# mcx/AgileRL

Hardware: AMD Instinct MI355X
Metric: population env-steps/sec + learner updates/sec, 8-agent PPO at 1/2/4/8 MI355X (higher is better)
Workload: dtype f32 (GAE carry f64); 1 GPU; config 2: one 8-agent PPO population sharded 8 agents per GPU, 128 vec envs per agent, T=16, batch 128, 4 epochs, MLP enc[64]->64 + heads[64] (shared encoder), tournament every 5 iterations; population=8, pop_per_gpu=8, num_envs=128, learn_step=2048, batch_size=128, update_epochs=4, learner=fused, parallelism=population-sharded x1

## Files before the change

agilerl_amd/csrc/learner.hip:

```cpp
#include <cmath>
#include <cstdlib>
#include <type_traits>

#include "agx_common.h"
#include "rollout.h"

namespace agx {

#ifndef AGX_LEARN_UNIFORM
#define AGX_LEARN_UNIFORM 1
#endif
#ifndef AGX_LEARN_RS2
#define AGX_LEARN_RS2 0
#endif
#ifndef AGX_LEARN_B2_TAGGED
#define AGX_LEARN_B2_TAGGED 1
#endif
#ifndef AGX_LEARN_B2_SWEEP1
#define AGX_LEARN_B2_SWEEP1 1
#endif
#ifndef AGX_LEARN_VEC_EARLY
#define AGX_LEARN_VEC_EARLY 1
#endif
#ifndef AGX_LEARN_STORE1
#define AGX_LEARN_STORE1 1
#endif

constexpr int kNT = 512;
constexpr int kNW = kNT / kWave;
constexpr int kSB = 32;
constexpr int kMaxSlot = 10;
constexpr int kMaxK = 16;
constexpr int kMaxPT = 32;
constexpr int kMaxA = 16;
constexpr int kMaxBlk = 28;

constexpr int kB2Words = 2 * kNW * kMaxK + 2;
constexpr size_t b2_words_off(size_t P) { return ((4 + kMaxK) * P + 1 + 3) / 4 * 4; }
typedef __attribute__((address_space(1))) unsigned long long gu64;

typedef unsigned v4u __attribute__((ext_vector_type(4)));

struct NetDims {
    int D, A, ne, eo[3], ha, hc;
};

struct Blk {
    int f0, len, rowlen, l0, ldst;
};

struct LearnPlan {
    int ok;
    int D, A, ne, ein[3], eout[3], eaff[3], lat, ha, hc, H, n;
    int f_ew[3], f_eb[3], f_eg[3], f_ebe[3];
    int f_aw, f_ab, f_ag, f_abe, f_aow, f_aob, f_cw, f_cb, f_cg, f_cbe, f_cow, f_cob;
    int l_ew[3], l_eld[3], l_eb[3], l_eg[3], l_ebe[3];
    int l_hw, l_hld, l_hb, l_hg, l_hbe;
    int l_aow, l_aold, l_aob, l_cow, l_cold, l_cob;
    int param_end;
    int l_x0, ld_x0, l_xe[3], ld_xe[3], l_re[3], l_xh, ld_xh, l_rh;
    int l_s1, l_s2, ld_s;
    int l_lg, l_dlg, l_dvb, l_val, l_row;
    int l_red, red_e[3], red_h, l_stat, l_stamp, l_b2x;
    int l_grad;
    int lds_floats, act_floats;
    int slab;
    int nt[6], ncol[6], slot0[6], nslot[6], nslots;
    int nblk;
    Blk blk[kMaxBlk];
};

constexpr int rup(int x, int m) { return (x + m - 1) / m * m; }

constexpr LearnPlan make_plan(NetDims d) {
    LearnPlan pl{};
    pl.ok = 0;
    pl.D = d.D;
    pl.A = d.A;
// ... 188 lines not shown
    if constexpr (W == 32)
        v = fmaxf(v, __builtin_bit_cast(float, __builtin_amdgcn_ds_swizzle(__builtin_bit_cast(int, v), 0x401f)));
    if constexpr (W == 64) {
        v = fmaxf(v, bcast<0x142, 0xa>(v, -__builtin_huge_valf()));
        v = fmaxf(v, bcast<0x143, 0xc>(v, -__builtin_huge_valf()));
        v = readlane_f(v, 63);
    }
    return v;
}
template <int W>
__device__ __forceinline__ int wrow(int lane, int wave) {
    return W == 64 ? wave : (W == 32 ? wave * 2 + (lane >> 5) : wave + kNW * (lane >> 4));
}
template <int SB>
constexpr int m_tiles() { return SB < 16 ? 1 : SB / 16; }
__device__ __forceinline__ float rowgroup_sum(float v) {
    v += __builtin_bit_cast(float, __builtin_amdgcn_ds_swizzle(__builtin_bit_cast(int, v), 0x401f));
    const int l = (int)(threadIdx.x & 63);
    return v + __builtin_bit_cast(float, __builtin_amdgcn_ds_bpermute((l ^ 32) << 2, __builtin_bit_cast(int, v)));
}
template <class T>
__device__ __forceinline__ T *in_vgpr(T *ptr) {
    asm volatile("" : "+v"(ptr));
    return ptr;
}
template <class T>
__device__ __forceinline__ T *to_sgpr(T *ptr) {
    const unsigned long long u = reinterpret_cast<unsigned long long>(ptr);
    const unsigned lo = __builtin_amdgcn_readfirstlane((unsigned)u);
    const unsigned hi = __builtin_amdgcn_readfirstlane((unsigned)(u >> 32));
    return reinterpret_cast<T *>(((unsigned long long)hi << 32) | lo);
}
__device__ __forceinline__ int vlane() {
    int v = (int)threadIdx.x;
    asm volatile("" : "+v"(v));
    return v & 63;
}
__device__ __forceinline__ int vtid() {
    int v = (int)threadIdx.x;
    asm volatile("" : "+v"(v));
    return v;
}
__device__ __forceinline__ int swave() {
    int w = __builtin_amdgcn_readfirstlane((int)threadIdx.x >> 6);
    asm volatile("" : "+s"(w));
    return w;
}
#define AGX_IDS                                             \
    const int lane = vlane(), wave = swave();               \
    const int lr16 = lane & 15, lq = lane >> 4;             \
    const int rrow = wave + kNW * lq, sub = lr16;           \
    (void)lr16, (void)lq, (void)rrow, (void)sub, (void)lane

__device__ __forceinline__ void block_sum2(float &a, float &b, float *stat, int slot, int lane, int wave) {
    a = row_sum(a);
    b = row_sum(b);
    const float wa = readlane_f(a, 0) + readlane_f(a, 16) + readlane_f(a, 32) + readlane_f(a, 48);
    const float wb = readlane_f(b, 0) + readlane_f(b, 16) + readlane_f(b, 32) + readlane_f(b, 48);
    if (lane == 0) {
        stat[slot * kNW + wave] = wa;
        stat[(slot + 1) * kNW + wave] = wb;
    }
    __syncthreads();
    float ta = 0.f, tb = 0.f;
    for (int i = 0; i < kNW; ++i) {
        ta += stat[slot * kNW + i];
        tb += stat[(slot + 1) * kNW + i];
    }
    a = ta;
    b = tb;
}

#ifndef AGX_MFMA_KB
#define AGX_MFMA_KB 16
#endif
template <int K, class FA, class FB>
__device__ __forceinline__ f4 mfma_tile(f4 acc, FA a, FB b) {
    const int lane = vlane();
    const int r = lane & 15, q = lane >> 4;
    constexpr int KB = K < AGX_MFMA_KB ? K : AGX_MFMA_KB;
    constexpr int NB = K / KB;
    static_assert(K % KB == 0 && KB % 4 == 0, "k batches");
    float av[2][KB / 4], bv[2][KB / 4];
#pragma unroll
    for (int j = 0; j < KB / 4; ++j) {
        av[0][j] = a(r, 4 * j + q);
        bv[0][j] = b(4 * j + q, r);
    }
#pragma unroll
    for (int i = 0; i < NB; ++i) {
        if (i + 1 < NB) {
#pragma unroll
            for (int j = 0; j < KB / 4; ++j) {
                av[(i + 1) & 1][j] = a(r, (i + 1) * KB + 4 * j + q);
                bv[(i + 1) & 1][j] = b((i + 1) * KB + 4 * j + q, r);
            }
        }
        __builtin_amdgcn_sched_barrier(0);
#pragma unroll
        for (int j = 0; j < KB / 4; ++j)
            acc = __builtin_amdgcn_mfma_f32_16x16x4f32(av[i & 1][j], bv[i & 1][j], acc, 0, 0, 0);
        __builtin_amdgcn_sched_barrier(0);
    }
    return acc;
}

template <class C>
__device__ __forceinline__ int flat_to_lds(int f) {
    constexpr LearnPlan pl = C::plan;
    int l = 0;
#pragma unroll
    for (int b = 0; b < pl.nblk; ++b) {
        constexpr int dummy = 0;
        (void)dummy;
        const Blk k = pl.blk[b];
        if (f >= k.f0 && f < k.f0 + k.len) {
            const int i = f - k.f0;
            l = k.l0 + (i / k.rowlen) * k.ldst + i % k.rowlen;
        }
    }
    return l;
}
template <class C>
// ... 223 lines not shown
#if AGX_LEARN_UNIFORM
    const int cs = (n4s + g.K - 1) / g.K;
    int oc0 = kk * cs < n4s ? kk * cs : n4s, oc1 = oc0 + cs < n4s ? oc0 + cs : n4s;
    const float inv_cs = 1.f / (float)cs;
#else
    int oc0 = n4s * kk / g.K, oc1 = n4s * (kk + 1) / g.K;
#endif
    int pc1 = oc1 < n4 ? oc1 : n4;
    constexpr int kUsed4 = JN > 0 ? JN : (n4 + kNT - 1) / kNT;
    static_assert(pl.param_end % 4 == 0 && pl.slab >= pl.param_end + 4 + 2 * kNW * kMaxK, "sum slab layout");
    static_assert(4 * kUsed4 <= kMaxPT, "owned slots");
    auto own_c = [&](int j) { return oc0 + vtid() + kNT * j; };
    const int jn_own = __builtin_amdgcn_readfirstlane((oc1 - oc0 + kNT - 1) / kNT);
    asm volatile("" : "+v"(oc0), "+v"(oc1), "+v"(pc1));
    float am[kMaxPT], av[kMaxPT];
    unsigned gbits = 0, vbits = 0;
#pragma unroll
    for (int i = 0; i < kMaxPT; ++i) {
        if (i >= 4 * kUsed4) {
            am[i] = av[i] = 0.f;
            continue;
        }
        const int c = own_c(i >> 2), l = 4 * c + (i & 3);
        int grp = 0;
        const int f = c < pc1 ? lds_to_flat<C>(l, grp) : -1;
        am[i] = f >= 0 ? gm[f] : 0.f;
        av[i] = f >= 0 ? gv[f] : 0.f;
        if (f >= 0) vbits |= 1u << i;
        if (grp) gbits |= 1u << i;
    }
    asm volatile("" : "+v"(vbits), "+v"(gbits));
    __syncthreads();

    constexpr int nmb_dummy = 0;
    (void)nmb_dummy;
    const int Bp = g.batch_p ? g.batch_p[p] : g.B;
    const int Ep = g.epochs_p ? g.epochs_p[p] : g.E;
    const float entp = g.ent_p ? g.ent_p[p] : g.ent;
    const int nmb = (int)((S + Bp - 1) / Bp);
    float loss_total = 0.f;
    double kl_total = 0.0;
    int n_done = 0, epochs_done = 0;
    const long long step0 = *step_v;
    double pb1 = pow((double)g.b1, (double)step0), pb2 = pow((double)g.b2, (double)step0);
    const float lr_p = g.lr[p];
    float *rowf = sm + pl.l_row;
    float *stat = sm + pl.l_stat;
    int *acts = reinterpret_cast<int *>(sm + pl.l_row + 4 * kSB);
    unsigned *legal = reinterpret_cast<unsigned *>(sm + pl.l_row + 5 * kSB);
    if (g.debug_stall && p == 0 && kk == 1) return;

    constexpr int kPreObs = (SB * pl.D + kNT - 1) / kNT;
    constexpr bool kPrefetch = kPreObs == 1;
    struct Pre {
        int e, mb, sb;
        float ob[kPreObs];
        unsigned rv;
    };
    const bool has_mask = g.gmask != nullptr;
    const int tid0 = vtid();
    const int rw_rr = tid0 < 4 * kSB ? tid0 % kSB : (tid0 < 5 * kSB ? tid0 - 4 * kSB : tid0 - 5 * kSB);
    const bool rw_on = tid0 < 6 * kSB;
    const unsigned *rw0 = in_vgpr(tid0 < 4 * kSB ? reinterpret_cast<const unsigned *>(g.grow) + ((size_t)p * 4 + tid0 / kSB) * S
                                  : (tid0 < 5 * kSB || !has_mask) ? reinterpret_cast<const unsigned *>(g.gact) + (size_t)p * S
                                                                   : g.gmask + (size_t)p * S);
    const size_t rw_es = (size_t)g.P * S * (tid0 < 4 * kSB ? 4 : 1);
    const float *ob0 = in_vgpr(g.gobs + (size_t)p * S * pl.D);
    const size_t ob_es = (size_t)g.P * S * pl.D;
    auto fetch = [&](int e_, int mb_, int sb_) {
        Pre r;
        r.e = e_;
        r.mb = mb_;
        r.sb = sb_;
        const int tid = vtid();
        const long long s0_ = (long long)mb_ * Bp;
        const int bsz_ = (int)((s0_ + Bp <= S) ? Bp : S - s0_);
        const int nrow_ = e_ >= Ep ? 0 : (bsz_ - sb_ < SB ? bsz_ - sb_ : SB);
        const size_t ee = (size_t)(e_ < Ep ? e_ : 0);
        const size_t row0 = (size_t)(s0_ + sb_);
        const float *eo = ob0 + ee * ob_es;
#pragma unroll
        for (int k = 0; k < kPreObs; ++k) {
            const int i = tid + k * kNT;
            r.ob[k] = eo[i < nrow_ * pl.D ? row0 * pl.D + i : 0];
        }
        r.rv = rw0[ee * rw_es + ((rw_on && rw_rr < nrow_) ? row0 + rw_rr : 0)];
        return r;
    };
    Pre pre{};
    if constexpr (kPrefetch) pre = fetch(0, 0, kk * SB);

    bool local = false;
    if (g.K > 1) {
        unsigned *xc = g.cnt + 3 * g.P + 1 + (size_t)p * kMaxK;
        if (tid == 0) {
            int x;
            asm volatile("s_getreg_b32 %0, hwreg(HW_REG_XCC_ID)" : "=s"(x));
            __hip_atomic_store(xc + kk, (unsigned)(x & 15) + 1u, __ATOMIC_RELAXED, __HIP_MEMORY_SCOPE_AGENT);
            asm volatile("s_waitcnt vmcnt(0)" ::: "memory");
            unsigned *ctr = g.cnt + 2 * g.P + 1 + p;
            __hip_atomic_fetch_add(ctr, 1u, __ATOMIC_RELAXED, __HIP_MEMORY_SCOPE_AGENT);
            unsigned spins = 0;
            int ok = 1;
            while (__hip_atomic_load(ctr, __ATOMIC_RELAXED, __HIP_MEMORY_SCOPE_AGENT) < (unsigned)g.K) {
                __builtin_amdgcn_s_sleep(1);
                if (++spins > kSpinMax) {
                    __hip_atomic_store(tmo_v, 1u, __ATOMIC_RELAXED, __HIP_MEMORY_SCOPE_AGENT);
                    if (err_v) __hip_atomic_fetch_or(err_v, 1u, __ATOMIC_RELAXED, __HIP_MEMORY_SCOPE_AGENT);
                    ok = 0;
                    break;
                }
            }
            stat[4 * kNW] = ok ? 1.f : 0.f;
        }
        __syncthreads();
        if (stat[4 * kNW] == 0.f) return;
        const int ln = vlane();
        const unsigned v = ln < g.K ? __hip_atomic_load(xc + ln, __ATOMIC_RELAXED, __HIP_MEMORY_SCOPE_AGENT) : 0u;
        const unsigned v0 = __builtin_amdgcn_readlane(v, 0);
        bool same = v0 != 0u;
        for (int q = 1; q < g.K; ++q) same = same && __builtin_amdgcn_readlane(v, q) == v0;
        local = same && !g.write_through;
    }

    float *slab_p = in_vgpr(g.slabs + (g.K > 1 ? (size_t)p * 2 * g.K * pl.slab : 0));
    float *sum_p = in_vgpr(g.sums + (g.K > 1 ? (size_t)p * 2 * pl.slab : 0));
    unsigned *ctr1 = in_vgpr(g.cnt + p);
    unsigned *ctr2 = in_vgpr(g.cnt + g.P + 1 + p);
    unsigned *ctr3 = in_vgpr(g.cnt + 3 * g.P + 1 + (size_t)g.P * kMaxK + p);
#if AGX_LEARN_B2_TAGGED
    unsigned long long *b2_p =
        in_vgpr(reinterpret_cast<unsigned long long *>(g.cnt + b2_words_off(g.P)) + (size_t)p * 2 * kB2Words);
    (void)ctr2;
#endif
    for (int e = 0; e < Ep; ++e) {
        for (int mb = 0; mb < nmb; ++mb) {
            const long long s0 = (long long)mb * Bp;
            const int bsz = (int)((s0 + Bp <= S) ? Bp : S - s0);
            const float inv_b = 1.f / (float)bsz;
            const int tid = vtid();
            f4 acc[kMaxSlot];
#pragma unroll
            for (int s = 0; s < kMaxSlot; ++s) acc[s] = f4{0.f, 0.f, 0.f, 0.f};
            const bool single = AGX_LEARN_STORE1 && kk * SB < bsz && kk * SB + g.K * SB >= bsz;
            if (!single)
                for (int i = tid; i < pl.l_stat - pl.l_red; i += kNT) sm[pl.l_red + i] = 0.f;
            float lsum = 0.f, klsum = 0.f;
            const int upd = e * nmb + mb;
            float *base = g.K > 1 ? to_sgpr(slab_p + (size_t)(upd & 1) * g.K * pl.slab) : nullptr;
            const auto slab_rsrc = __builtin_amdgcn_make_buffer_rsrc(base + (size_t)kk * pl.slab, 0,
                                                                     __builtin_amdgcn_readfirstlane(pl.slab * 4),
                                                                     0x00020000);
            auto emit_tiles = [&](auto gc, auto fn) {
                constexpr int gg = decltype(gc)::value;
                AGX_IDS;
#pragma unroll
                for (int j = 0; j < pl.nslot[gg]; ++j) {
                    const int t = wave + kNW * j;
                    if (t < pl.nt[gg]) {
                        const int o0 = (t / pl.ncol[gg]) * 16, i0 = (t % pl.ncol[gg]) * 16;
                        const int col = i0 + lr16;
#pragma unroll
                        for (int i = 0; i < 4; ++i) {
                            const int o = o0 + lq * 4 + i;
                            const float x = acc[pl.slot0[gg] + j][i];
                            if constexpr (gg < pl.ne) {
                                if (col < pl.ein[gg]) fn(pl.l_ew[gg] + o * pl.l_eld[gg] + col, x);
                            } else if constexpr (gg == pl.ne) {
                                fn(pl.l_hw + o * pl.l_hld + col, x);
                            } else if constexpr (gg == pl.ne + 1) {
                                if (o < pl.A) {
                                    if (col < pl.ha) fn(pl.l_aow + o * pl.l_aold + col, x);
                                    else if (col == pl.ha) fn(pl.l_aob + o, x);
                                }
                            } else {
                                if (o == 0) {
                                    if (col < pl.hc) fn(pl.l_cow + col, x);
                                    else if (col == pl.hc) fn(pl.l_cob, x);
                                }
                            }
                        }
                    }
                }
            };
            auto put_l = [&](int l, float x) {
                __builtin_amdgcn_raw_buffer_store_b32(__builtin_bit_cast(unsigned, x), slab_rsrc, l * 4, 0, 0);
            };
            auto put_w = [&](int l, float x) {
                __builtin_amdgcn_raw_buffer_store_b32(__builtin_bit_cast(unsigned, x), slab_rsrc, l * 4, 0, 16);
            };
            auto slab_put = [&](int l, float x) {
                if (local) put_l(l, x);
                else put_w(l, x);
            };
            auto emit_slab = [&](auto gc) {
                if (local) emit_tiles(gc, put_l);
                else emit_tiles(gc, put_w);
            };
            auto vdump = [&](auto Lc, auto put) {
                constexpr int L = decltype(Lc)::value;
                constexpr int F = L < pl.ne ? pl.eout[L < pl.ne ? L : 0] : pl.H;
                constexpr int nv = (L < pl.ne && !pl.eaff[L < pl.ne ? L : 0]) ? 1 : 3;
                constexpr int red = L < pl.ne ? pl.red_e[L < pl.ne ? L : 0] : pl.red_h;
                const int tid = vtid();
#pragma unroll
                for (int rnd = 0; rnd < (nv * F + kNT - 1) / kNT; ++rnd) {
                    const int idx = tid + rnd * kNT;
                    if (idx >= nv * F) break;
                    const int k = idx / F, j = idx % F;
                    float pv[kNW];
#pragma unroll
                    for (int w = 0; w < kNW; ++w) pv[w] = sm[pl.l_red + red + (k * kNW + w) * F + j];
                    float x = 0.f;
#pragma unroll
                    for (int w = 0; w < kNW; ++w) x += pv[w];
                    int l;
                    if constexpr (L < pl.ne) {
                        l = (k == 0 ? pl.l_eb[L < pl.ne ? L : 0] : (k == 1 ? pl.l_eg[L < pl.ne ? L : 0] : pl.l_ebe[L < pl.ne ? L : 0])) + j;
                    } else {
                        l = (k == 0 ? pl.l_hb : (k == 1 ? pl.l_hg : pl.l_hbe)) + j;
                    }
                    put(l, x);
                }
            };
            auto vdump_slab = [&](auto Lc) {
                if (local) vdump(Lc, put_l);
                else vdump(Lc, put_w);
            };
            const auto sum_rsrc = __builtin_amdgcn_make_buffer_rsrc(
                g.K > 1 ? to_sgpr(sum_p + (size_t)(upd & 1) * pl.slab) : nullptr, 0,
                __builtin_amdgcn_readfirstlane(pl.slab * 4), 0x00020000);
            (void)sum_rsrc;
            auto partner_sync = [&](unsigned *ctr, unsigned target, int st0, int st1) -> bool {
                asm volatile("s_waitcnt vmcnt(0)" ::: "memory");
                __syncthreads();
                const int tid = vtid();
                if (tid == 0) {
                    const unsigned before = __hip_atomic_fetch_add(ctr, 1u, __ATOMIC_RELAXED, __HIP_MEMORY_SCOPE_AGENT);
                    AGX_STAMP(st0);
                    unsigned spins = 0;
                    int ok = 1;
                    while (before + 1u < target &&
                           __hip_atomic_load(ctr, __ATOMIC_RELAXED, __HIP_MEMORY_SCOPE_AGENT) < target) {
                        __builtin_amdgcn_s_sleep(1);
                        if (++spins > kSpinMax) {
                            __hip_atomic_store(tmo_v, 1u, __ATOMIC_RELAXED, __HIP_MEMORY_SCOPE_AGENT);
                            if (err_v) __hip_atomic_fetch_or(err_v, 1u, __ATOMIC_RELAXED, __HIP_MEMORY_SCOPE_AGENT);
                            ok = 0;
                            break;
                        }
                    }
                    asm volatile("s_waitcnt vmcnt(0)" ::: "memory");
                    stat[4 * kNW] = ok ? 1.f : 0.f;
                    AGX_STAMP(st1);
                }
                __syncthreads();
                return stat[4 * kNW] != 0.f;
            };
            const bool direct = g.K > 1;
            const bool vec_early = AGX_LEARN_VEC_EARLY && direct;

            for (int sb = kk * SB; sb < bsz; sb += g.K * SB) {
                const bool last_sb = sb + g.K * SB >= bsz;
                const int nrow = bsz - sb < SB ? bsz - sb : SB;
                const int jsb = (sb / SB) / g.K;
                const int stb = jsb < 4 ? jsb * 16 : 80;
                const int tid = vtid();
                AGX_STAMP(stb + 0);
                {
                    auto commit = [&](const Pre &x) {
                        __builtin_amdgcn_s_waitcnt(0x0F70);
#pragma unroll
                        for (int k = 0; k < kPreObs; ++k) {
                            const int i = tid + k * kNT;
                            if (i < SB * pl.D) sm[pl.l_x0 + (i / pl.D) * pl.ld_x0 + i % pl.D] = i < nrow * pl.D ? x.ob[k] : 0.f;
                        }
                        constexpr int npad = pl.ld_x0 - pl.D;
#pragma unroll
                        for (int k = 0; k < (SB * npad + kNT - 1) / kNT; ++k) {
                            const int i = tid + k * kNT;
                            if (i < SB * npad) sm[pl.l_x0 + (i / npad) * pl.ld_x0 + pl.D + i % npad] = 0.f;
                        }
                        if (tid < 4 * kSB) rowf[tid] = tid % kSB < nrow ? __builtin_bit_cast(float, x.rv) : 0.f;
                        else if (tid < 5 * kSB) acts[tid - 4 * kSB] = tid - 4 * kSB < nrow ? (int)x.rv : 0;
                        else if (tid < 6 * kSB) legal[tid - 5 * kSB] = (has_mask && tid - 5 * kSB < nrow) ? x.rv : 0xffffffffu;
                    };
                    if constexpr (!kPrefetch) {
                        commit(fetch(e, mb, sb));
                    } else {
                        if (pre.e != e || pre.mb != mb || pre.sb != sb) pre = fetch(e, mb, sb);
                        commit(pre);
                        AGX_STAMP(stb + 4);
                        int ne = e, nm = mb, ns = sb + g.K * SB;
                        if (ns >= bsz) {
                            ns = kk * SB;
                            if (++nm >= nmb) {
                                nm = 0;
                                ++ne;
                            }
                        }
                        pre = fetch(ne, nm, ns);
                        AGX_STAMP(stb + 5);
                    }
                }
                __syncthreads();
                AGX_STAMP(stb + 1);

                fw.trunk([&](int k) { AGX_STAMP(stb + k); });
                AGX_STAMP(stb + 2);

                {
                    constexpr int W = (SB == 8 && pl.H % 64 == 0 && pl.ha % 64 == 0)
                                          ? 64
                                          : ((SB <= 16 && pl.H % 32 == 0 && pl.ha % 32 == 0) ? 32 : 16);
                    const int lane = vlane(), wave = swave();
                    const int sub = lane & (W - 1);
                    const int r = wrow<W>(lane, wave);
                    constexpr int F = pl.H, split = pl.ha, NC = F / W, NA = pl.A;
                    constexpr int F0 = split, F1 = F - split;
                    const int a = sub;
                    auto swz16 = [](float v) {
                        return __builtin_bit_cast(float, __builtin_amdgcn_ds_swizzle(__builtin_bit_cast(int, v), 0x401f));
                    };
                    auto rsum = [&](float v) { return wrow_sum<W>(v); };
                    auto rmax = [&](float v) { return wrow_max<W>(v); };
                    const bool rl = r < SB;
                    const bool live = rl && r < nrow;
                    float z[NC], xh[NC];
                    float s0 = 0.f, s1 = 0.f;
#pragma unroll
                    for (int i = 0; i < NC; ++i) {
                        z[i] = rl ? sm[pl.l_s2 + r * pl.ld_s + sub + W * i] : 0.f;
                        if (W * i < split) s0 += z[i];
                        else s1 += z[i];
                    }
                    const float m0 = rsum(s0) * (1.f / (float)F0);
                    const float m1 = rsum(s1) * (1.f / (float)F1);
                    float v0 = 0.f, v1 = 0.f;
#pragma unroll
                    for (int i = 0; i < NC; ++i) {
                        if (W * i < split) v0 += (z[i] - m0) * (z[i] - m0);
                        else v1 += (z[i] - m1) * (z[i] - m1);
                    }
                    const float r0 = 1.f / sqrtf(rsum(v0) / (float)F0 + 1e-5f);
                    const float r1 = 1.f / sqrtf(rsum(v1) / (float)F1 + 1e-5f);
                    float pa[NA], pv = 0.f;
#pragma unroll
                    for (int k = 0; k < NA; ++k) pa[k] = 0.f;
#pragma unroll
                    for (int i = 0; i < NC; ++i) {
                        const int j = sub + W * i;
                        xh[i] = W * i < split ? (z[i] - m0) * r0 : (z[i] - m1) * r1;
                        const float y = relu(xh[i] * sm[pl.l_hg + j] + sm[pl.l_hbe + j]);
                        if (rl) sm[pl.l_s1 + r * pl.ld_s + j] = y;
                        if (W * i < split) {
#pragma unroll
                            for (int k = 0; k < NA; ++k) pa[k] += y * sm[pl.l_aow + k * pl.l_aold + j];
                        } else {
// ... 79 lines not shown
                            a1 += dxh[i];
                            a2 += dxh[i] * xh[i];
                        } else {
                            c1 += dxh[i];
                            c2 += dxh[i] * xh[i];
                        }
                    }
                    const float rs0 = rl ? r0 : 0.f, rs1 = rl ? r1 : 0.f;
                    const float ma1 = rsum(a1) * (1.f / (float)F0), ma2 = rsum(a2) * (1.f / (float)F0);
                    const float mc1 = rsum(c1) * (1.f / (float)F1), mc2 = rsum(c2) * (1.f / (float)F1);
                    float *rd = sm + pl.l_red + pl.red_h;
                    float cs[3][NC];
#pragma unroll
                    for (int i = 0; i < NC; ++i) {
                        const int j = sub + W * i;
                        const bool g0 = W * i < split;
                        const float dz = (g0 ? rs0 : rs1) * (dxh[i] - (g0 ? ma1 : mc1) - xh[i] * (g0 ? ma2 : mc2));
                        if (rl) sm[pl.l_s2 + r * pl.ld_s + j] = dz;
                        cs[0][i] = rl ? dz : 0.f;
                        cs[1][i] = dyp[i] * xh[i];
                        cs[2][i] = dyp[i];
                    }
                    if constexpr (W == 16) {
#pragma unroll
                        for (int k = 0; k < 3; ++k)
#pragma unroll
                            for (int i = 0; i < NC; ++i) cs[k][i] += swz16(cs[k][i]);
                    }
                    if constexpr (W == 32 || (W == 16 && SB > 16)) {
#pragma unroll
                        for (int k = 0; k < 3; ++k)
#pragma unroll
                            for (int i = 0; i < NC; ++i)
                                cs[k][i] += __builtin_bit_cast(
                                    float, __builtin_amdgcn_ds_bpermute((lane ^ 32) << 2, __builtin_bit_cast(int, cs[k][i])));
                    }
                    if (lane < W) {
                        if (single) {
#pragma unroll
                            for (int k = 0; k < 3; ++k)
#pragma unroll
                                for (int i = 0; i < NC; ++i) rd[(k * kNW + wave) * F + sub + W * i] = cs[k][i] + 0.f;
                        } else {
#pragma unroll
                            for (int k = 0; k < 3; ++k) {
                                float o[NC];
#pragma unroll
                                for (int i = 0; i < NC; ++i) o[i] = rd[(k * kNW + wave) * F + sub + W * i];
#pragma unroll
                                for (int i = 0; i < NC; ++i) rd[(k * kNW + wave) * F + sub + W * i] = o[i] + cs[k][i];
                            }
                        }
                    }
                }
                __syncthreads();
                AGX_STAMP(stb + 3);
                if (vec_early && last_sb) vdump_slab(IC(pl.ne));

                auto ln_bwd = [&](auto Fc, auto dybc, auto ldyc, auto xbc, auto ldxc, auto rbc, auto gbc, auto bbc,
                                  auto redc, auto affc) {
                    constexpr int F = decltype(Fc)::value;
                    constexpr int dyb = decltype(dybc)::value, ldy = decltype(ldyc)::value;
                    constexpr int xb = decltype(xbc)::value, ldx = decltype(ldxc)::value;
                    constexpr int rb = decltype(rbc)::value, gb = decltype(gbc)::value, bb = decltype(bbc)::value;
                    constexpr int red = decltype(redc)::value;
                    constexpr bool aff = decltype(affc)::value;
                    constexpr int W = (SB == 8 && F % 64 == 0) ? 64 : ((SB <= 16 && F % 32 == 0) ? 32 : 16);
                    constexpr int NC = F / W;
                    const int lane = vlane(), wave = swave();
                    const int sub = lane & (W - 1);
                    const int r = wrow<W>(lane, wave);
                    const bool rl = r < SB;
                    float xh[NC], dxh[NC], dyp[NC];
                    float a1 = 0.f, a2 = 0.f;
                    const float rs0 = rl ? sm[rb + 2 * r] : 0.f;
#pragma unroll
                    for (int i = 0; i < NC; ++i) {
                        const int j = sub + W * i;
                        const float dy = rl ? sm[dyb + r * ldy + j] : 0.f;
                        xh[i] = rl ? sm[xb + r * ldx + j] : 0.f;
                        const float gam = aff ? sm[gb + j] : 1.f;
                        const float y = aff ? xh[i] * gam + sm[bb + j] : xh[i];
                        dyp[i] = y > 0.f ? dy : 0.f;
                        dxh[i] = dyp[i] * gam;
                        a1 += dxh[i];
                        a2 += dxh[i] * xh[i];
                    }
                    const float ma1 = wrow_sum<W>(a1) * (1.f / (float)F), ma2 = wrow_sum<W>(a2) * (1.f / (float)F);
                    float *rd = sm + pl.l_red + red;
                    constexpr int NV = aff ? 3 : 1;
                    float cs[NV][NC];
#pragma unroll
                    for (int i = 0; i < NC; ++i) {
                        const int j = sub + W * i;
                        const float dz = rs0 * (dxh[i] - ma1 - xh[i] * ma2);
                        if (rl) sm[pl.l_s2 + r * pl.ld_s + j] = dz;
                        cs[0][i] = rl ? dz : 0.f;
                        if constexpr (aff) {
                            cs[1][i] = dyp[i] * xh[i];
                            cs[2][i] = dyp[i];
                        }
                    }
                    if constexpr (W == 16) {
#pragma unroll
                        for (int k = 0; k < NV; ++k)
#pragma unroll
                            for (int i = 0; i < NC; ++i)
                                cs[k][i] += __builtin_bit_cast(
                                    float, __builtin_amdgcn_ds_swizzle(__builtin_bit_cast(int, cs[k][i]), 0x401f));
// ... 85 lines not shown
                    }
                }
                __syncthreads();
                AGX_STAMP(stb + 6);

                auto enc_bwd = [&](auto Lc) {
                    constexpr int L = decltype(Lc)::value;
                    constexpr int fin = pl.ein[L], fout = pl.eout[L];
                    AGX_IDS;
                    constexpr int dyb = L == pl.ne - 1 ? pl.l_xh : pl.l_s1;
                    constexpr int ldy = L == pl.ne - 1 ? pl.ld_xh : pl.ld_s;
                    ln_bwd(IC(fout), IC(dyb), IC(ldy), IC(pl.l_xe[L]), IC(pl.ld_xe[L]), IC(pl.l_re[L]), IC(pl.l_eg[L]),
                           IC(pl.l_ebe[L]), IC(pl.red_e[L]), BC(pl.eaff[L] != 0));
                    __syncthreads();
                    if (vec_early && last_sb) vdump_slab(Lc);
                    constexpr bool in_aff = L > 0 && pl.eaff[L > 0 ? L - 1 : 0];
                    constexpr int xb = L == 0 ? pl.l_x0 : pl.l_xe[L > 0 ? L - 1 : 0];
                    constexpr int ldx = L == 0 ? pl.ld_x0 : pl.ld_xe[L > 0 ? L - 1 : 0];
                    constexpr int gbase = L > 0 ? pl.l_eg[L > 0 ? L - 1 : 0] : 0;
                    constexpr int bbase = L > 0 ? pl.l_ebe[L > 0 ? L - 1 : 0] : 0;
#pragma unroll
                    for (int j = 0; j < pl.nslot[L]; ++j) {
                        const int t = wave + kNW * j;
                        if (t < pl.nt[L]) {
                            const int o0 = (t / pl.ncol[L]) * 16, i0 = (t % pl.ncol[L]) * 16;
                            const int col = i0 + lr16;
                            const bool cv = col < fin;
                            const float gam = (in_aff && cv) ? sm[gbase + col] : 1.f;
                            const float bet = (in_aff && cv) ? sm[bbase + col] : 0.f;
                            acc[pl.slot0[L] + j] = mfma_tile<SB>(
                                acc[pl.slot0[L] + j], [&](int m, int k) { return sm[pl.l_s2 + k * pl.ld_s + o0 + m]; },
                                [&](int k, int n) {
                                    const float x = sm[xb + k * ldx + i0 + n];
                                    if constexpr (L == 0) return x;
                                    else return cv ? relu(x * gam + bet) : 0.f;
                                });
                        }
                    }
                    if (direct && last_sb) emit_slab(IC(L));
                    if constexpr (L > 0) {
                        constexpr int MT = m_tiles<SB>();
                        constexpr int nt = MT * (fin / 16);
                        for (int t = wave; t < nt; t += kNW) {
                            const int m0 = (t % MT) * 16, n0 = (t / MT) * 16;
                            f4 c = f4{0.f, 0.f, 0.f, 0.f};
                            c = mfma_tile<fout>(c, [&](int m, int k) { return sm[pl.l_s2 + (m0 + m) * pl.ld_s + k]; },
                                                [&](int k, int n) { return sm[pl.l_ew[L] + k * pl.l_eld[L] + n0 + n]; });
                            if (SB >= 16 || lq * 4 < SB) {
#pragma unroll
                                for (int i = 0; i < 4; ++i) sm[pl.l_s1 + (m0 + lq * 4 + i) * pl.ld_s + n0 + lr16] = c[i];
                            }
                        }
                    }
                    __syncthreads();
                };
                if constexpr (pl.ne == 3) enc_bwd(IC(2));
                enc_bwd(IC(1));
                enc_bwd(IC(0));
                AGX_STAMP(stb + 7);
            }

            float *G = sm + pl.l_grad;
            auto gput = [&](int l, float x) { G[l] = x; };
            if (!direct) {
                emit_tiles(IC(0), gput);
                emit_tiles(IC(1), gput);
                if constexpr (pl.ne == 3) emit_tiles(IC(2), gput);
                emit_tiles(IC(pl.ne), gput);
                emit_tiles(IC(pl.ne + 1), gput);
                emit_tiles(IC(pl.ne + 2), gput);
            } else if (kk * SB >= bsz) {
                emit_slab(IC(0));
                emit_slab(IC(1));
                if constexpr (pl.ne == 3) emit_slab(IC(2));
                emit_slab(IC(pl.ne));
                emit_slab(IC(pl.ne + 1));
                emit_slab(IC(pl.ne + 2));
            }
            auto vdump_all = [&](auto put) {
                vdump(IC(0), put);
                vdump(IC(1), put);
                if constexpr (pl.ne == 3) vdump(IC(2), put);
                vdump(IC(pl.ne), put);
            };
            if (!direct) vdump_all(gput);
            else if (!vec_early || kk * SB >= bsz) {
                if (local) vdump_all(put_l);
                else vdump_all(put_w);
            }
            AGX_STAMP(64 + 9);
            __syncthreads();
            float lmb = lsum, klmb = klsum;
            {
                AGX_IDS;
                block_sum2(lmb, klmb, stat, 2, lane, wave);
            }
            float gr[kMaxPT];
            constexpr int NQ = (2 * kNW * KM + 63) / 64;
            float vq[NQ];
            if (g.K > 1) {
                if (tid == 0) {
                    slab_put(pl.param_end, lmb);
                    slab_put(pl.param_end + 1, klmb);
                }
                if (!partner_sync(ctr1, (unsigned)(g.K * (upd + 1)), 64 + 11, 64 + 12)) return;
#if AGX_LEARN_B2_TAGGED
                gu64 *const b2w = (gu64 *)(b2_p + (size_t)(upd & 1) * kB2Words);
                const unsigned long long b2tag = (unsigned long long)(unsigned)(upd + 1) << 32;
                auto b2_store = [&](gu64 *w, unsigned v) {
                    if (local) __hip_atomic_store(w, b2tag | v, __ATOMIC_RELAXED, __HIP_MEMORY_SCOPE_WORKGROUP);
                    else __hip_atomic_store(w, b2tag | v, __ATOMIC_RELAXED, __HIP_MEMORY_SCOPE_AGENT);
                };
                auto put_loss = [&](f4 t) {
                    const float lw = t[0], kw = t[1];
                    b2_store(b2w + 2 * kNW * kMaxK, __builtin_bit_cast(unsigned, lw));
                    b2_store(b2w + 2 * kNW * kMaxK + 1, __builtin_bit_cast(unsigned, kw));
                };
#else
                auto put_loss = [&](f4 t) {
                    if (local) __builtin_amdgcn_raw_buffer_store_b128(__builtin_bit_cast(v4u, t), sum_rsrc, n4 * 16, 0, 0);
                    else __builtin_amdgcn_raw_buffer_store_b128(__builtin_bit_cast(v4u, t), sum_rsrc, n4 * 16, 0, 16);
                };
#endif
                {
                    const int tid = vtid();
                    const auto rs = __builtin_amdgcn_make_buffer_rsrc(
                        base, 0, __builtin_amdgcn_readfirstlane(g.K * pl.slab * 4), 0x00020000);
                    bool rs_done = false;
#if AGX_LEARN_RS2
                    if constexpr (JN == 1) {
                        if (oc1 - oc0 <= kNT / 2) {
                            constexpr int KH = KM / 2;
                            const int h = tid >= kNT / 2 ? 1 : 0;
                            const int c = oc0 + (tid & (kNT / 2 - 1));
                            const int cl = c < oc1 ? c : oc0;
                            f4 x[KH];
#pragma unroll
                            for (int q = 0; q < KH; ++q) {
                                const int qq = KH * h + q, qs = qq < g.K ? qq : g.K - 1;
                                const f4 v = __builtin_bit_cast(
                                    f4, __builtin_amdgcn_raw_buffer_load_b128(rs, (qs * pl.slab + 4 * cl) * 4, 0, 16));
                                x[q] = qq < g.K ? v : f4{0.f, 0.f, 0.f, 0.f};
                            }
                            f4 t = x[0];
#pragma unroll
                            for (int q = 1; q < KH; ++q) t += x[q];
                            f4 *xch = reinterpret_cast<f4 *>(sm + pl.l_x0);
                            if (h) xch[tid - kNT / 2] = t;
                            __syncthreads();
                            if (!h) {
                                t += xch[tid];
                                if (c == n4) put_loss(t);
                            }
#pragma unroll
                            for (int cc = 0; cc < 4; ++cc) gr[cc] = (!h && c < pc1) ? t[cc] : 0.f;
                            rs_done = true;
                        }
                    }
// ... 61 lines not shown
                    unsigned lo[NQ], ll = 0u;
#if AGX_LEARN_B2_SWEEP1
                    unsigned *b2x = reinterpret_cast<unsigned *>(sm + pl.l_b2x);
                    bool swept = true;
                    if (swave() == 0) {
#endif
                    for (unsigned spins = 0;;) {
                        unsigned long long x[NQ];
#pragma unroll
                        for (int q = 0; q < NQ; ++q)
                            x[q] = __hip_atomic_load(b2w + 64 * q + lane, __ATOMIC_RELAXED, __HIP_MEMORY_SCOPE_AGENT);
                        const unsigned long long xl =
                            __hip_atomic_load(b2w + 2 * kNW * kMaxK + (lane & 1), __ATOMIC_RELAXED, __HIP_MEMORY_SCOPE_AGENT);
                        unsigned bad = (unsigned)(xl >> 32) ^ tag;
                        ll = (unsigned)xl;
#pragma unroll
                        for (int q = 0; q < NQ; ++q) {
                            bad |= lane + 64 * q < np ? (unsigned)(x[q] >> 32) ^ tag : 0u;
                            lo[q] = (unsigned)x[q];
                        }
                        if (__all(bad == 0u)) break;
                        __builtin_amdgcn_s_sleep(1);
                        if (++spins > kSpinMax) {
                            __hip_atomic_store(tmo_v, 1u, __ATOMIC_RELAXED, __HIP_MEMORY_SCOPE_AGENT);
                            if (err_v) __hip_atomic_fetch_or(err_v, AGX_LEARN_ERR_TIMEOUT, __ATOMIC_RELAXED, __HIP_MEMORY_SCOPE_AGENT);
#if AGX_LEARN_B2_SWEEP1
                            swept = false;
                            break;
#else
                            return;
#endif
                        }
                    }
#if AGX_LEARN_B2_SWEEP1
#pragma unroll
                        for (int q = 0; q < NQ; ++q) b2x[lane + 64 * q] = lo[q];
                        if (lane < 2) b2x[2 * kNW * kMaxK + lane] = ll;
                        if (lane == 0) stat[4 * kNW] = swept ? 1.f : 0.f;
                    }
                    __syncthreads();
                    if (stat[4 * kNW] == 0.f) return;
#pragma unroll
                    for (int q = 0; q < NQ; ++q) lo[q] = b2x[lane + 64 * q];
                    ll = b2x[2 * kNW * kMaxK + (lane & 1)];
#endif
#pragma unroll
                    for (int q = 0; q < NQ; ++q) vq[q] = lane + 64 * q < np ? __builtin_bit_cast(float, lo[q]) : 0.f;
                    lmb = __builtin_bit_cast(float, __builtin_amdgcn_readlane(ll, 0));
                    klmb = __builtin_bit_cast(float, __builtin_amdgcn_readlane(ll, 1));
                }
                AGX_STAMP(64 + 15);
#else
                AGX_STAMP(64 + 13);
                if (!partner_sync(ctr2, (unsigned)(g.K * (upd + 1)), 64 + 8, 64 + 15)) return;
                {
                    const int lane = vlane();
                    const int np = 2 * kNW * g.K;
#pragma unroll
                    for (int q = 0; q < NQ; ++q) {
                        const float x = __builtin_bit_cast(
                            float, __builtin_amdgcn_raw_buffer_load_b32(sum_rsrc, (pl.param_end + 4 + 64 * q + lane) * 4, 0, 16));
                        vq[q] = lane + 64 * q < np ? x : 0.f;
                    }
                }
                const unsigned lw = __builtin_amdgcn_raw_buffer_load_b32(sum_rsrc, pl.param_end * 4, 0, 16);
                const unsigned kw = __builtin_amdgcn_raw_buffer_load_b32(sum_rsrc, (pl.param_end + 1) * 4, 0, 16);
                lmb = __builtin_bit_cast(float, __builtin_amdgcn_readfirstlane(lw));
                klmb = __builtin_bit_cast(float, __builtin_amdgcn_readfirstlane(kw));
#endif
            }

            float t0 = 0.f, t1 = 0.f;
            if (!direct) {
                const f4 *G4 = reinterpret_cast<const f4 *>(G);
#pragma unroll
                for (int j = 0; j < kUsed4; ++j) {
                    const int c = own_c(j);
                    const f4 x = c < pc1 ? G4[c] : f4{0.f, 0.f, 0.f, 0.f};
#pragma unroll
                    for (int cc = 0; cc < 4; ++cc) gr[4 * j + cc] = x[cc];
                }
                float n0 = 0.f, n1 = 0.f;
#pragma unroll
                for (int i = 0; i < 4 * kUsed4; ++i) {
                    const bool valid = (vbits >> i) & 1u, crit = (gbits >> i) & 1u;
                    gr[i] = valid ? gr[i] : 0.f;
                    const float x2 = gr[i] * gr[i];
                    n1 += crit ? x2 : 0.f;
                    n0 += crit ? 0.f : x2;
                }
                AGX_IDS;
                {
                    const float r0 = row_sum(n0), r1 = row_sum(n1);
                    const float w0 = readlane_f(r0, 0) + readlane_f(r0, 16) + readlane_f(r0, 32) + readlane_f(r0, 48);
                    const float w1 = readlane_f(r1, 0) + readlane_f(r1, 16) + readlane_f(r1, 32) + readlane_f(r1, 48);
                    if (lane == 0) {
                        stat[wave] = w0;
                        stat[kNW + wave] = w1;
                    }
                }
                __syncthreads();
                for (int i = 0; i < kNW; ++i) {
                    t0 += stat[i];
                    t1 += stat[kNW + i];
                }
            } else {
                const int lane = vlane();
// ... 10 lines not shown
            AGX_STAMP(64 + 14);
            const float c0 = g.max_norm > 0.f ? fminf(g.max_norm / (sqrtf(t0) + 1e-6f), 1.f) : 1.f;
            const float c1 = g.max_norm > 0.f ? fminf(g.max_norm / (sqrtf(t1) + 1e-6f), 1.f) : 1.f;
            pb1 *= (double)g.b1;
            pb2 *= (double)g.b2;
            const float bc1 = (float)(1.0 - pb1);
            const float bc2s = (float)sqrt(1.0 - pb2);
            const float step_size = lr_p / bc1;
            const float inv_bc2s = 1.f / bc2s;
            f4 pv[kMaxPT / 4];
            f4 *sm4 = reinterpret_cast<f4 *>(sm);
#pragma unroll
            for (int j = 0; j < kUsed4; ++j) {
                const int c = own_c(j);
                pv[j] = (j < jn_own && c < pc1) ? sm4[c] : f4{0.f, 0.f, 0.f, 0.f};
            }
            const float ob1 = 1.f - g.b1, ob2 = 1.f - g.b2;
#pragma unroll
            for (int j = 0; j < kUsed4; ++j) {
                if (j >= jn_own) break;
                f4 gc, m, v;
#pragma unroll
                for (int c = 0; c < 4; ++c) {
                    const int i = 4 * j + c;
                    gc[c] = ((gbits >> i) & 1u) ? c1 : c0;
                    m[c] = am[i];
                    v[c] = av[i];
                }
                gc = f4{gr[4 * j], gr[4 * j + 1], gr[4 * j + 2], gr[4 * j + 3]} * gc;
                m = m + ob1 * (gc - m);
                v = v * g.b2 + ob2 * gc * gc;
                f4 r;
#pragma unroll
                for (int c = 0; c < 4; ++c) r[c] = __builtin_amdgcn_sqrtf(v[c]);
                r = r * inv_bc2s + g.eps;
#pragma unroll
                for (int c = 0; c < 4; ++c) r[c] = __builtin_amdgcn_rcpf(r[c]);
                const f4 nv = pv[j] - step_size * (m * r);
#pragma unroll
                for (int c = 0; c < 4; ++c) {
                    am[4 * j + c] = m[c];
                    av[4 * j + c] = v[c];
                }
                const int c = own_c(j);
                if (c < pc1) {
                    sm4[c] = nv;
                    if (direct) {
                        if (local) __builtin_amdgcn_raw_buffer_store_b128(__builtin_bit_cast(v4u, nv), slab_rsrc, c * 16, 0, 0);
                        else __builtin_amdgcn_raw_buffer_store_b128(__builtin_bit_cast(v4u, nv), slab_rsrc, c * 16, 0, 16);
                    }
                }
            }
            if (direct) {
                if (!partner_sync(ctr3, (unsigned)(g.K * (upd + 1)), 64 + 0,
                                  64 + 1))
                    return;
                const int tid = vtid();
                const auto rs = __builtin_amdgcn_make_buffer_rsrc(
                    base, 0, __builtin_amdgcn_readfirstlane(g.K * pl.slab * 4), 0x00020000);
#if AGX_LEARN_UNIFORM
                constexpr int NR = (n4 + kNT - 1) / kNT;
                f4 x[NR];
#pragma unroll
                for (int j = 0; j < NR; ++j) {
                    const int c0 = tid + kNT * j, c = c0 < n4 ? c0 : n4 - 1;
                    const int q = (int)(((float)c + 0.5f) * inv_cs);
                    x[j] = __builtin_bit_cast(f4, __builtin_amdgcn_raw_buffer_load_b128(rs, (q * pl.slab + 4 * c) * 4, 0, 16));
                }
#pragma unroll
                for (int j = 0; j < NR; ++j) {
                    const int c = tid + kNT * j;
                    const int q = (int)(((float)c + 0.5f) * inv_cs);
                    if (c < n4 && q != kk) sm4[c] = x[j];
                }
#else
                const int span = (n4s + g.K - 1) / g.K + 1;
                for (int r0 = 0; r0 < span; r0 += kNT) {
                    f4 x[KM];
                    int cq[KM];
#pragma unroll
                    for (int q = 0; q < KM; ++q) {
                        const int qc0 = (int)((long long)n4s * q / g.K), qc1 = (int)((long long)n4s * (q + 1) / g.K);
                        const int c = qc0 + tid + r0;
                        cq[q] = (q < g.K && q != kk && c < qc1 && c < n4) ? c : -1;
                        x[q] = cq[q] >= 0 ? __builtin_bit_cast(f4, __builtin_amdgcn_raw_buffer_load_b128(
                                                                        rs, (q * pl.slab + 4 * c) * 4, 0, 16))
                                          : f4{0.f, 0.f, 0.f, 0.f};
                    }
#pragma unroll
                    for (int q = 0; q < KM; ++q)
                        if (cq[q] >= 0) sm4[cq[q]] = x[q];
                }
#endif
                AGX_STAMP(64 + 2);
            }
            __syncthreads();
            AGX_STAMP(64 + 10);
        }
        ++epochs_done;
        {
            const unsigned long long tb = __builtin_bit_cast(unsigned long long, tkl_v);
            const unsigned thi = __builtin_amdgcn_readfirstlane((unsigned)(tb >> 32));
            const unsigned tlo = __builtin_amdgcn_readfirstlane((unsigned)tb);
            const double tkl = __builtin_bit_cast(double, ((unsigned long long)thi << 32) | tlo);
            if (tkl > 0.0 && kl_total / (double)n_done > tkl) break;
        }
    }

// ... 596 lines not shown
```

Measured before the change: 10.02 million env-steps/s.

## Stage next minibatch inputs into LDS while waiting on partner sync

Moves the LDS commit of the prefetched next-minibatch observations and row data into the partner_sync wait for the parameter exchange. The atomic poll runs on the last wave while the other waves stage the data, so the next iteration can skip its commit and barrier. It also adds an optional tail-early loss reduction, disabled by default, that removes a barrier before the partner sync. This adds complexity around which waves own shared memory and when the prefetch is consumed, with some risk of races on the staged buffers.

```diff
diff --git a/agilerl_amd/csrc/learner.hip b/agilerl_amd/csrc/learner.hip
--- a/agilerl_amd/csrc/learner.hip
+++ b/agilerl_amd/csrc/learner.hip
@@ -24,6 +24,12 @@
 #endif
 #ifndef AGX_LEARN_STORE1
 #define AGX_LEARN_STORE1 1
+#endif
+#ifndef AGX_LEARN_STAGE_EARLY
+#define AGX_LEARN_STAGE_EARLY 1
+#endif
+#ifndef AGX_LEARN_TAIL_EARLY
+#define AGX_LEARN_TAIL_EARLY 0
 #endif
 
 constexpr int kNT = 512;
@@ -318,7 +324,7 @@
     const int rrow = wave + kNW * lq, sub = lr16;           \
     (void)lr16, (void)lq, (void)rrow, (void)sub, (void)lane
 
-__device__ __forceinline__ void block_sum2(float &a, float &b, float *stat, int slot, int lane, int wave) {
+__device__ __forceinline__ void block_sum2_put(float a, float b, float *stat, int slot, int lane, int wave) {
     a = row_sum(a);
     b = row_sum(b);
     const float wa = readlane_f(a, 0) + readlane_f(a, 16) + readlane_f(a, 32) + readlane_f(a, 48);
@@ -327,7 +333,8 @@
         stat[slot * kNW + wave] = wa;
         stat[(slot + 1) * kNW + wave] = wb;
     }
-    __syncthreads();
+}
+__device__ __forceinline__ void block_sum2_get(float &a, float &b, const float *stat, int slot) {
     float ta = 0.f, tb = 0.f;
     for (int i = 0; i < kNW; ++i) {
         ta += stat[slot * kNW + i];
@@ -335,6 +342,11 @@
     }
     a = ta;
     b = tb;
+}
+__device__ __forceinline__ void block_sum2(float &a, float &b, float *stat, int slot, int lane, int wave) {
+    block_sum2_put(a, b, stat, slot, lane, wave);
+    __syncthreads();
+    block_sum2_get(a, b, stat, slot);
 }
 
 #ifndef AGX_MFMA_KB
@@ -664,6 +676,9 @@
 
     constexpr int kPreObs = (SB * pl.D + kNT - 1) / kNT;
     constexpr bool kPrefetch = kPreObs == 1;
+    constexpr int kStageT0 = SB * pl.D > 6 * kSB ? SB * pl.D : 6 * kSB;
+    constexpr int kStageT = kStageT0 > SB * (pl.ld_x0 - pl.D) ? kStageT0 : SB * (pl.ld_x0 - pl.D);
+    constexpr bool kStage = AGX_LEARN_STAGE_EARLY && kPrefetch && kStageT <= kNT - kWave;
     struct Pre {
         int e, mb, sb;
         float ob[kPreObs];
@@ -745,12 +760,17 @@
         in_vgpr(reinterpret_cast<unsigned long long *>(g.cnt + b2_words_off(g.P)) + (size_t)p * 2 * kB2Words);
     (void)ctr2;
 #endif
+    int staged_v = 0;
+    asm volatile("" : "+v"(staged_v));
     for (int e = 0; e < Ep; ++e) {
         for (int mb = 0; mb < nmb; ++mb) {
             const long long s0 = (long long)mb * Bp;
             const int bsz = (int)((s0 + Bp <= S) ? Bp : S - s0);
             const float inv_b = 1.f / (float)bsz;
             const int tid = vtid();
+            const bool was_staged = kStage && __builtin_amdgcn_readfirstlane(staged_v) != 0;
+            staged_v = 0;
+            asm volatile("" : "+v"(staged_v));
             f4 acc[kMaxSlot];
 #pragma unroll
             for (int s = 0; s < kMaxSlot; ++s) acc[s] = f4{0.f, 0.f, 0.f, 0.f};
@@ -843,13 +863,23 @@
                 g.K > 1 ? to_sgpr(sum_p + (size_t)(upd & 1) * pl.slab) : nullptr, 0,
                 __builtin_amdgcn_readfirstlane(pl.slab * 4), 0x00020000);
             (void)sum_rsrc;
-            auto partner_sync = [&](unsigned *ctr, unsigned target, int st0, int st1) -> bool {
-                asm volatile("s_waitcnt vmcnt(0)" ::: "memory");
+            auto partner_sync = [&](unsigned *ctr, unsigned target, int st0, int st1, auto pollc, auto under) -> bool {
+                constexpr int PT = decltype(pollc)::value;
+                if constexpr (PT == 0) asm volatile("s_waitcnt vmcnt(0)" ::: "memory");
+                else __builtin_amdgcn_s_waitcnt(0x0F70);
                 __syncthreads();
-                const int tid = vtid();
-                if (tid == 0) {
-                    const unsigned before = __hip_atomic_fetch_add(ctr, 1u, __ATOMIC_RELAXED, __HIP_MEMORY_SCOPE_AGENT);
+                const int rtid = vtid();
+                unsigned before = 0u;
+                if (rtid == PT) {
+                    before = __hip_atomic_fetch_add(ctr, 1u, __ATOMIC_RELAXED, __HIP_MEMORY_SCOPE_AGENT);
+                    const int tid = 0;
+                    (void)tid;
                     AGX_STAMP(st0);
+                }
+                under();
+                if (rtid == PT) {
+                    const int tid = 0;
+                    (void)tid;
                     unsigned spins = 0;
                     int ok = 1;
                     while (before + 1u < target &&
@@ -871,6 +901,48 @@
             };
             const bool direct = g.K > 1;
             const bool vec_early = AGX_LEARN_VEC_EARLY && direct;
+            int tail_v = (AGX_LEARN_TAIL_EARLY && direct && kk * SB < bsz) ? 1 : 0;
+            asm volatile("" : "+v"(tail_v));
+            auto tail_early = [&]() -> bool {
+                if constexpr (!AGX_LEARN_TAIL_EARLY) return false;
+                else return __builtin_amdgcn_readfirstlane(tail_v) != 0;
+            };
+            auto commit = [&](const Pre &x, int nr) {
+                const int tid = vtid();
+#pragma unroll
+                for (int k = 0; k < kPreObs; ++k) {
+                    const int i = tid + k * kNT;
+                    if (i < SB * pl.D) sm[pl.l_x0 + (i / pl.D) * pl.ld_x0 + i % pl.D] = i < nr * pl.D ? x.ob[k] : 0.f;
+                }
+                constexpr int npad = pl.ld_x0 - pl.D;
+#pragma unroll
+                for (int k = 0; k < (SB * npad + kNT - 1) / kNT; ++k) {
+                    const int i = tid + k * kNT;
+                    if (i < SB * npad) sm[pl.l_x0 + (i / npad) * pl.ld_x0 + pl.D + i % npad] = 0.f;
+                }
+                if (tid < 4 * kSB) rowf[tid] = tid % kSB < nr ? __builtin_bit_cast(float, x.rv) : 0.f;
+                else if (tid < 5 * kSB) acts[tid - 4 * kSB] = tid - 4 * kSB < nr ? (int)x.rv : 0;
+                else if (tid < 6 * kSB) legal[tid - 5 * kSB] = (has_mask && tid - 5 * kSB < nr) ? x.rv : 0xffffffffu;
+            };
+            auto fetch_after = [&](int e_, int mb_, int sb_, int bsz_, auto loadc) {
+                int ne = e_, nm = mb_, ns = sb_ + g.K * SB;
+                if (ns >= bsz_) {
+                    ns = kk * SB;
+                    if (++nm >= nmb) {
+                        nm = 0;
+                        ++ne;
+                    }
+                }
+                if constexpr (decltype(loadc)::value) {
+                    return fetch(ne, nm, ns);
+                } else {
+                    Pre r = pre;
+                    r.e = ne;
+                    r.mb = nm;
+                    r.sb = ns;
+                    return r;
+                }
+            };
 
             for (int sb = kk * SB; sb < bsz; sb += g.K * SB) {
                 const bool last_sb = sb + g.K * SB >= bsz;
@@ -879,43 +951,24 @@
                 const int stb = jsb < 4 ? jsb * 16 : 80;
                 const int tid = vtid();
                 AGX_STAMP(stb + 0);
-                {
-                    auto commit = [&](const Pre &x) {
+                if (!was_staged) {
+                    if constexpr (!kPrefetch) {
+                        const Pre x = fetch(e, mb, sb);
                         __builtin_amdgcn_s_waitcnt(0x0F70);
-#pragma unroll
-                        for (int k = 0; k < kPreObs; ++k) {
-                            const int i = tid + k * kNT;
-                            if (i < SB * pl.D) sm[pl.l_x0 + (i / pl.D) * pl.ld_x0 + i % pl.D] = i < nrow * pl.D ? x.ob[k] : 0.f;
-                        }
-                        constexpr int npad = pl.ld_x0 - pl.D;
-#pragma unroll
-                        for (int k = 0; k < (SB * npad + kNT - 1) / kNT; ++k) {
-                            const int i = tid + k * kNT;
-                            if (i < SB * npad) sm[pl.l_x0 + (i / npad) * pl.ld_x0 + pl.D + i % npad] = 0.f;
-                        }
-                        if (tid < 4 * kSB) rowf[tid] = tid % kSB < nrow ? __builtin_bit_cast(float, x.rv) : 0.f;
-                        else if (tid < 5 * kSB) acts[tid - 4 * kSB] = tid - 4 * kSB < nrow ? (int)x.rv : 0;
-                        else if (tid < 6 * kSB) legal[tid - 5 * kSB] = (has_mask && tid - 5 * kSB < nrow) ? x.rv : 0xffffffffu;
-                    };
-                    if constexpr (!kPrefetch) {
-                        commit(fetch(e, mb, sb));
+                        commit(x, nrow);
                     } else {
                         if (pre.e != e || pre.mb != mb || pre.sb != sb) pre = fetch(e, mb, sb);
-                        commit(pre);
+                        __builtin_amdgcn_s_waitcnt(0x0F70);
+                        commit(pre, nrow);
                         AGX_STAMP(stb + 4);
-                        int ne = e, nm = mb, ns = sb + g.K * SB;
-                        if (ns >= bsz) {
-                            ns = kk * SB;
-                            if (++nm >= nmb) {
-                                nm = 0;
-                                ++ne;
-                            }
-                        }
-                        pre = fetch(ne, nm, ns);
+                        pre = fetch_after(e, mb, sb, bsz, BC(true));
                         AGX_STAMP(stb + 5);
                     }
-                }
-                __syncthreads();
+                    __syncthreads();
+                } else {
+                    AGX_STAMP(stb + 4);
+                    AGX_STAMP(stb + 5);
+                }
                 AGX_STAMP(stb + 1);
 
                 fw.trunk([&](int k) { AGX_STAMP(stb + k); });
@@ -1101,9 +1154,16 @@
                             }
                         }
                     }
+                    if (last_sb && tail_early()) block_sum2_put(lsum, klsum, stat, 2, lane, wave);
                 }
                 __syncthreads();
                 AGX_STAMP(stb + 3);
+                if (last_sb && tail_early() && tid == 0) {
+                    float lw, kw;
+                    block_sum2_get(lw, kw, stat, 2);
+                    slab_put(pl.param_end, lw);
+                    slab_put(pl.param_end + 1, kw);
+                }
                 if (vec_early && last_sb) vdump_slab(IC(pl.ne));
 
                 auto ln_bwd = [&](auto Fc, auto dybc, auto ldyc, auto xbc, auto ldxc, auto rbc, auto gbc, auto bbc,
@@ -1295,7 +1355,7 @@
                             }
                         }
                     }
-                    __syncthreads();
+                    if (!(L == 0 && last_sb && tail_early())) __syncthreads();
                 };
                 if constexpr (pl.ne == 3) enc_bwd(IC(2));
                 enc_bwd(IC(1));
@@ -1332,9 +1392,9 @@
                 else vdump_all(put_w);
             }
             AGX_STAMP(64 + 9);
-            __syncthreads();
             float lmb = lsum, klmb = klsum;
-            {
+            if (!tail_early()) {
+                __syncthreads();
                 AGX_IDS;
                 block_sum2(lmb, klmb, stat, 2, lane, wave);
             }
@@ -1342,11 +1402,11 @@
             constexpr int NQ = (2 * kNW * KM + 63) / 64;
             float vq[NQ];
             if (g.K > 1) {
-                if (tid == 0) {
+                if (!tail_early() && tid == 0) {
                     slab_put(pl.param_end, lmb);
                     slab_put(pl.param_end + 1, klmb);
                 }
-                if (!partner_sync(ctr1, (unsigned)(g.K * (upd + 1)), 64 + 11, 64 + 12)) return;
+                if (!partner_sync(ctr1, (unsigned)(g.K * (upd + 1)), 64 + 11, 64 + 12, IC(0), [] {})) return;
 #if AGX_LEARN_B2_TAGGED
                 gu64 *const b2w = (gu64 *)(b2_p + (size_t)(upd & 1) * kB2Words);
                 const unsigned long long b2tag = (unsigned long long)(unsigned)(upd + 1) << 32;
@@ -1514,7 +1574,7 @@
                 AGX_STAMP(64 + 15);
 #else
                 AGX_STAMP(64 + 13);
-                if (!partner_sync(ctr2, (unsigned)(g.K * (upd + 1)), 64 + 8, 64 + 15)) return;
+                if (!partner_sync(ctr2, (unsigned)(g.K * (upd + 1)), 64 + 8, 64 + 15, IC(0), [] {})) return;
                 {
                     const int lane = vlane();
                     const int np = 2 * kNW * g.K;
@@ -1631,8 +1691,32 @@
                 }
             }
             if (direct) {
-                if (!partner_sync(ctr3, (unsigned)(g.K * (upd + 1)), 64 + 0,
-                                  64 + 1))
+                if (!partner_sync(ctr3, (unsigned)(g.K * (upd + 1)), 64 + 0, 64 + 1, IC(kStage ? kNT - kWave : 0), [&] {
+                        if constexpr (kStage) {
+                            int ne1 = e, nm1 = mb + 1;
+                            if (nm1 >= nmb) {
+                                nm1 = 0;
+                                ++ne1;
+                            }
+                            asm volatile("" : "+v"(ne1), "+v"(nm1));
+                            const long long s1 = (long long)nm1 * Bp;
+                            const int bsz1 = (int)((s1 + Bp <= S) ? Bp : S - s1);
+                            const bool stage_next =
+                                single && ne1 < Ep && kk * SB < bsz1 && kk * SB + g.K * SB >= bsz1;
+                            if (stage_next) {
+                                if (swave() < (kStageT + kWave - 1) / kWave) {
+                                    commit(pre, bsz1 - kk * SB < SB ? bsz1 - kk * SB : SB);
+                                    AGX_STAMP(64 + 4);
+                                    pre = fetch_after(ne1, nm1, kk * SB, bsz1, BC(true));
+                                    AGX_STAMP(64 + 5);
+                                } else {
+                                    pre = fetch_after(ne1, nm1, kk * SB, bsz1, BC(false));
+                                }
+                                staged_v = 1;
+                                asm volatile("" : "+v"(staged_v));
+                            }
+                        }
+                    }))
                     return;
                 const int tid = vtid();
                 const auto rs = __builtin_amdgcn_make_buffer_rsrc(
```

Measured after the change: 10.31 million env-steps/s, median of 6. +2.8%, better.
